# evenrose/CMDIAD

Hardware: AMD Instinct MI355X
Metric: images/sec end-to-end (extract+distill+kNN score) (higher is better)
Workload: dtype bf16; 1 GPU; configs[1]: DINO ViT-B/8 + Point-MAE predict (DoubleRGBPointFeatures: both modalities are extracted, this method has no distillation step at test time; the `mtfi_step` leg times the method that has one), 224x224 RGB + 24576-point clouds (1024 groups x 128), batch 32/GPU, bagel-sized banks (xyz 76518x768, rgb 19129x768); batch_per_gpu=32, rotating_input_batches=4, bank=single, hip_graphs=True, search_operands=bf16 (fp32 accumulate, exact fp32 re-score of the winner), weights=seeded random init (no checkpoints offline)

## Files before the change

cmdiad_amd/csrc/fps.hip:

```cpp
#include "common.h"
#include "launch.h"

namespace {

constexpr int kThreads = 1024;
constexpr int kWaves = kThreads / 64;
constexpr int kMaxRegPoints = 512 * 56;

__device__ __forceinline__ unsigned long long wave_max_u64(unsigned long long v)
{
#pragma unroll
    for (int m = 32; m >= 1; m >>= 1) {
        unsigned long long o = shfl_xor_u64(v, m);
        v = o > v ? o : v;
    }
    return v;
}

__device__ __forceinline__ unsigned long long fps_key(float v, int idx)
{
    return v < 0.0f ? 0ull : (((unsigned long long)__float_as_uint(v) << 32) | (0xFFFFFFFFu - (unsigned)idx));
}

#ifdef CMDIAD_AB_VARIANTS
#include "ab/fps_reg.inc"
#endif


__device__ __forceinline__ unsigned dpp_max_u32(unsigned v)
{
    unsigned o;
    o = (unsigned)__builtin_amdgcn_update_dpp(0, (int)v, 0xB1, 0xF, 0xF, false); v = o > v ? o : v;
    o = (unsigned)__builtin_amdgcn_update_dpp(0, (int)v, 0x4E, 0xF, 0xF, false); v = o > v ? o : v;
    o = (unsigned)__builtin_amdgcn_update_dpp(0, (int)v, 0x141, 0xF, 0xF, false); v = o > v ? o : v;
    o = (unsigned)__builtin_amdgcn_update_dpp(0, (int)v, 0x140, 0xF, 0xF, false); v = o > v ? o : v;
    const unsigned a = __builtin_amdgcn_readlane(v, 0), b = __builtin_amdgcn_readlane(v, 16);
    const unsigned c = __builtin_amdgcn_readlane(v, 32), d = __builtin_amdgcn_readlane(v, 48);
    const unsigned ab = a > b ? a : b, cd = c > d ? c : d;
    return ab > cd ? ab : cd;
}

__device__ __forceinline__ unsigned dpp_min_u32(unsigned v)
{
    unsigned o;
    o = (unsigned)__builtin_amdgcn_update_dpp(0, (int)v, 0xB1, 0xF, 0xF, false); v = o < v ? o : v;
    o = (unsigned)__builtin_amdgcn_update_dpp(0, (int)v, 0x4E, 0xF, 0xF, false); v = o < v ? o : v;
    o = (unsigned)__builtin_amdgcn_update_dpp(0, (int)v, 0x141, 0xF, 0xF, false); v = o < v ? o : v;
    o = (unsigned)__builtin_amdgcn_update_dpp(0, (int)v, 0x140, 0xF, 0xF, false); v = o < v ? o : v;
    const unsigned a = __builtin_amdgcn_readlane(v, 0), b = __builtin_amdgcn_readlane(v, 16);
    const unsigned c = __builtin_amdgcn_readlane(v, 32), d = __builtin_amdgcn_readlane(v, 48);
    const unsigned ab = a < b ? a : b, cd = c < d ? c : d;
    return ab < cd ? ab : cd;
}

template <int kThreads, int PPT, bool TAIL>
__device__ __forceinline__ void fps_pk_body(const float* __restrict__ p, const int n, const int G, int32_t* __restrict__ out,
                                            float* __restrict__ cen, float4* __restrict__ lds_pts, const int lds_cap,
                                            float* __restrict__ temp)
{
    static_assert(PPT % 2 == 0, "two points per packed operation");
    constexpr int kWaves = kThreads / 64, H = PPT / 2, R = PPT * kThreads;
    __shared__ unsigned long long s_key[2][kWaves];
    const int tid = threadIdx.x;

    f32x2 px[H], py[H], pz[H], t[H];
#pragma unroll
    for (int h = 0; h < H; ++h)
#pragma unroll
        for (int e = 0; e < 2; ++e) {
            const int k = (2 * h + e) * kThreads + tid;
            const int kk = max(min(k, n - 1), 0);
            const float x = p[kk * 3 + 0], y = p[kk * 3 + 1], z = p[kk * 3 + 2];
            px[h][e] = x; py[h][e] = y; pz[h][e] = z;
            const float mag = (x * x + y * y) + z * z;
            t[h][e] = (k < n && !(mag <= 1e-3f)) ? 1e10f : -__builtin_inff();
        }
    const int n_lds = TAIL ? min(max(n - R, 0), lds_cap) : 0;
    const int g0 = R + n_lds;
    if constexpr (TAIL) {
        for (int e = tid; e < n_lds; e += kThreads) {
            const int k = R + e;
            const float x = p[k * 3 + 0], y = p[k * 3 + 1], z = p[k * 3 + 2];
            const float mag = (x * x + y * y) + z * z;
            lds_pts[e] = float4{x, y, z, !(mag <= 1e-3f) ? 1e10f : -__builtin_inff()};
        }
        for (int k = g0 + tid; k < n; k += kThreads) {
            const float x = p[k * 3 + 0], y = p[k * 3 + 1], z = p[k * 3 + 2];
            const float mag = (x * x + y * y) + z * z;
            temp[k] = !(mag <= 1e-3f) ? 1e10f : -__builtin_inff();
        }
    }

    int old = 0;
    if (tid == 0 && G > 0) {
        out[0] = 0;
        if (cen) { cen[0] = p[0]; cen[1] = p[1]; cen[2] = p[2]; }
    }
    for (int j = 1; j < G; ++j) {
        const int so = __builtin_amdgcn_readfirstlane(old);
        const float x1 = p[so * 3 + 0], y1 = p[so * 3 + 1], z1 = p[so * 3 + 2];
        const f32x2 X1 = {x1, x1}, Y1 = {y1, y1}, Z1 = {z1, z1};
        int best = 0;
#pragma unroll
        for (int h = 0; h < H; ++h) {
            const f32x2 dx = px[h] - X1, dy = py[h] - Y1, dz = pz[h] - Z1;
            const f32x2 d = (dx * dx + dy * dy) + dz * dz;
            const int a = min((int)__float_as_uint(d[0]), (int)__float_as_uint(t[h][0]));
            const int c = min((int)__float_as_uint(d[1]), (int)__float_as_uint(t[h][1]));
            t[h][0] = __uint_as_float((unsigned)a);
            t[h][1] = __uint_as_float((unsigned)c);
            best = max(best, max(a, c));
        }
        int tb = -1, ti = 0;
        if constexpr (TAIL) {
            for (int e = tid; e < n_lds; e += kThreads) {
                const float4 q = lds_pts[e];
                const float dx = q.x - x1, dy = q.y - y1, dz = q.z - z1;
                const float d = (dx * dx + dy * dy) + dz * dz;
                const int a = min((int)__float_as_uint(d), (int)__float_as_uint(q.w));
                lds_pts[e].w = __uint_as_float((unsigned)a);
                if (a > tb) { tb = a; ti = R + e; }
            }
            for (int k = g0 + tid; k < n; k += kThreads) {
                const float dx = p[k * 3] - x1, dy = p[k * 3 + 1] - y1, dz = p[k * 3 + 2] - z1;
                const float d = (dx * dx + dy * dy) + dz * dz;
                const int a = min((int)__float_as_uint(d), (int)__float_as_uint(temp[k]));
                temp[k] = __uint_as_float((unsigned)a);
                if (a > tb) { tb = a; ti = k; }
            }
        }
        const unsigned wbits = dpp_max_u32((unsigned)max(best, tb));
        int slot = -1;
        unsigned long long lanes = 0ull;
#pragma unroll
        for (int c0 = 0; c0 < PPT; c0 += 8) {
            unsigned long long m[8];
            unsigned long long any = 0ull;
#pragma unroll
            for (int e = 0; e < 8; ++e) {
                const int sl = c0 + e;
                m[e] = sl < PPT ? __ballot(__float_as_uint(t[sl >> 1][sl & 1]) == wbits) : 0ull;
                any |= m[e];
            }
            if (any != 0ull) {
#pragma unroll
                for (int e = 7; e >= 0; --e)
                    if (m[e] != 0ull) { slot = c0 + e; lanes = m[e]; }
                break;
            }
        }
        unsigned long long key = 0ull;
        if (slot >= 0) {
            const int besti = slot * kThreads + (tid & ~63) + (__ffsll((long long)lanes) - 1);
            key = ((unsigned long long)wbits << 32) | (0xFFFFFFFFu - (unsigned)besti);
        } else if constexpr (TAIL) {
            const unsigned cand = dpp_min_u32(tb == (int)wbits ? (unsigned)ti : 0xFFFFFFFFu);
            if (cand != 0xFFFFFFFFu) key = ((unsigned long long)wbits << 32) | (0xFFFFFFFFu - cand);
        }
        const int buf = j & 1;
        if ((tid & 63) == 0) s_key[buf][tid >> 6] = key;
        __syncthreads();
        unsigned long long m = s_key[buf][0];
#pragma unroll
        for (int w = 1; w < kWaves; ++w) {
            const unsigned long long o = s_key[buf][w];
            m = o > m ? o : m;
        }
        old = m == 0ull ? 0 : (int)(0xFFFFFFFFu - (unsigned)(m & 0xFFFFFFFFull));
        if (tid == 0) {
            out[j] = old;
            if (cen) { cen[j * 3 + 0] = p[old * 3 + 0]; cen[j * 3 + 1] = p[old * 3 + 1]; cen[j * 3 + 2] = p[old * 3 + 2]; }
        }
    }
}

template <int kThreads, int PPT>
__global__ __launch_bounds__(kThreads) void fps_pk_kernel(const float* __restrict__ xyz,
                                                          const int32_t* __restrict__ n_valid, int N, int G,
                                                          int32_t* __restrict__ idx_out,
                                                          float* __restrict__ center_out)
{
    const int b = blockIdx.x;
    fps_pk_body<kThreads, PPT, false>(xyz + (size_t)b * N * 3, n_valid ? n_valid[b] : N, G, idx_out + (size_t)b * G,
                                      center_out ? center_out + (size_t)b * G * 3 : nullptr, nullptr, 0, nullptr);
}

constexpr int kRaggedThreads = 512;
constexpr int kMaxLdsPoints = 9728;
__global__ __launch_bounds__(kRaggedThreads) void fps_ragged_kernel(const float* __restrict__ xyz,
                                                                    const int32_t* __restrict__ n_valid, int N, int G,
                                                                    int lds_cap, float* __restrict__ temp_ws,
                                                                    int32_t* __restrict__ idx_out, float* __restrict__ center_out)
{
    extern __shared__ __attribute__((aligned(16))) float4 fps_lds[];
    const int b = blockIdx.x;
    const int n = __builtin_amdgcn_readfirstlane(n_valid ? n_valid[b] : N);
    const float* p = xyz + (size_t)b * N * 3;
    int32_t* out = idx_out + (size_t)b * G;
    float* cen = center_out ? center_out + (size_t)b * G * 3 : nullptr;
    if (n <= kRaggedThreads * 40) fps_pk_body<kRaggedThreads, 40, false>(p, n, G, out, cen, nullptr, 0, nullptr);
    else if (n <= kRaggedThreads * 48) fps_pk_body<kRaggedThreads, 48, false>(p, n, G, out, cen, nullptr, 0, nullptr);
    else if (n <= kRaggedThreads * 56) fps_pk_body<kRaggedThreads, 56, false>(p, n, G, out, cen, nullptr, 0, nullptr);
    else fps_pk_body<kRaggedThreads, 56, true>(p, n, G, out, cen, fps_lds, lds_cap, temp_ws ? temp_ws + (size_t)b * N : nullptr);
}

#ifdef CMDIAD_AB_VARIANTS
__global__ __launch_bounds__(kThreads) void fps_mem_kernel(const float* __restrict__ xyz,
                                                           const int32_t* __restrict__ n_valid, int N, int G,
                                                           float* __restrict__ temp_ws,
                                                           int32_t* __restrict__ idx_out,
                                                           float* __restrict__ center_out)
{
    __shared__ unsigned long long s_key[2][kWaves];
    const int b = blockIdx.x;
    const int tid = threadIdx.x;
    const int n = n_valid ? n_valid[b] : N;
    const float* p = xyz + (size_t)b * N * 3;
    float* temp = temp_ws + (size_t)b * N;
    int32_t* out = idx_out + (size_t)b * G;
    float* cen = center_out ? center_out + (size_t)b * G * 3 : nullptr;

    for (int k = tid; k < n; k += kThreads) {
        const float x = p[k * 3], y = p[k * 3 + 1], z = p[k * 3 + 2];
        const float mag = (x * x + y * y) + z * z;
        temp[k] = !(mag <= 1e-3f) ? 1e10f : -__builtin_inff();
    }
    int old = 0;
    if (tid == 0 && G > 0) {
        out[0] = 0;
        if (cen) { cen[0] = p[0]; cen[1] = p[1]; cen[2] = p[2]; }
    }
    for (int j = 1; j < G; ++j) {
        const int so = __builtin_amdgcn_readfirstlane(old);
        const float x1 = p[so * 3 + 0], y1 = p[so * 3 + 1], z1 = p[so * 3 + 2];
        float best = -1.0f;
        int besti = 0;
        for (int k = tid; k < n; k += kThreads) {
            const float dx = p[k * 3] - x1, dy = p[k * 3 + 1] - y1, dz = p[k * 3 + 2] - z1;
            const float d = (dx * dx + dy * dy) + dz * dz;
            const float d2 = fminf(d, temp[k]);
            temp[k] = d2;
            const bool gt = d2 > best;
            best = gt ? d2 : best;
            besti = gt ? k : besti;
        }
        unsigned long long key = wave_max_u64(fps_key(best, besti));
        const int buf = j & 1;
        if ((tid & 63) == 0) s_key[buf][tid >> 6] = key;
        __syncthreads();
        unsigned long long m = s_key[buf][0];
#pragma unroll
        for (int w = 1; w < kWaves; ++w) {
            const unsigned long long o = s_key[buf][w];
            m = o > m ? o : m;
        }
        old = m == 0ull ? 0 : (int)(0xFFFFFFFFu - (unsigned)(m & 0xFFFFFFFFull));
        if (tid == 0) {
            out[j] = old;
            if (cen) { cen[j * 3 + 0] = p[old * 3 + 0]; cen[j * 3 + 1] = p[old * 3 + 1]; cen[j * 3 + 2] = p[old * 3 + 2]; }
        }
    }
}

#endif

}

struct FpsWs { float* min_d; size_t total; };
static FpsWs fps_layout(void* base, int B, int N)
{
    Carve c(base);
    return {c.take<float>(N > kMaxRegPoints + kMaxLdsPoints ? (size_t)B * (size_t)N : 0), c.total()};
}

extern "C" size_t cmdiad_fps_workspace_bytes(int B, int N) { return fps_layout(nullptr, B, N).total; }

extern "C" int cmdiad_fps(const float* xyz, const int32_t* n_valid, int B, int N, int G, int32_t* idx_out,
                          float* center_out, void* workspace, size_t workspace_bytes, cmdiad_stream_t stream)
{
    CMDIAD_REQUIRE(xyz && idx_out, CMDIAD_ERR_ARG, "cmdiad_fps: null pointer");
    CMDIAD_REQUIRE(B >= 0 && N > 0 && G >= 0, CMDIAD_ERR_ARG, "cmdiad_fps: bad sizes B=%d N=%d G=%d", B, N, G);
    if (B == 0 || G == 0) return CMDIAD_OK;
    hipStream_t s = (hipStream_t)stream;
#ifdef CMDIAD_AB_VARIANTS
    const bool pk = !env_is("CMDIAD_FPS_PK", '0');
    const bool ragged_ok = !env_is("CMDIAD_FPS_RAGGED", '0');
#define FPS_LAUNCH(T, P)                                                                                                      \
    do {                                                                                                                      \
        if (pk) hipLaunchKernelGGL((fps_pk_kernel<T, P>), dim3(B), dim3(T), 0, s, xyz, n_valid, N, G, idx_out, center_out);   \
        else hipLaunchKernelGGL((fps_reg_kernel<T, P>), dim3(B), dim3(T), 0, s, xyz, n_valid, N, G, idx_out, center_out);     \
    } while (0)
#else
    const bool ragged_ok = true;
#define FPS_LAUNCH(T, P) hipLaunchKernelGGL((fps_pk_kernel<T, P>), dim3(B), dim3(T), 0, s, xyz, n_valid, N, G, idx_out, center_out)
#endif
    const bool ragged = ragged_ok && N > 1024 * 16 && (n_valid != nullptr || N > kMaxRegPoints);
    if (ragged) {
        const int lds_cap = N > kMaxRegPoints ? (N - kMaxRegPoints < kMaxLdsPoints ? N - kMaxRegPoints : kMaxLdsPoints) : 0;
        const FpsWs L = fps_layout(workspace, B, N);
        if (const int rc = workspace_ok("cmdiad_fps", workspace, workspace_bytes, L.total)) return rc;
        if (const int rc = launch_lds<fps_ragged_kernel>("cmdiad_fps", dim3(B), dim3(kRaggedThreads), (size_t)lds_cap * sizeof(float4), s, xyz, n_valid,
                                                         N, G, lds_cap, L.total ? L.min_d : nullptr, idx_out, center_out))
            return rc;
    }
    else if (N <= 1024 * 4) FPS_LAUNCH(1024, 4);
    else if (N <= 1024 * 8) FPS_LAUNCH(1024, 8);
    else if (N <= 1024 * 16) FPS_LAUNCH(1024, 16);
    else if (N <= 512 * 40) FPS_LAUNCH(512, 40);
    else if (N <= 512 * 48) FPS_LAUNCH(512, 48);
    else if (N <= 512 * 56) FPS_LAUNCH(512, 56);
#undef FPS_LAUNCH
    else {
#ifdef CMDIAD_AB_VARIANTS
        Carve c(workspace);
        float* const min_d = c.take<float>((size_t)B * (size_t)N);
        if (const int rc = workspace_ok("cmdiad_fps", workspace, workspace_bytes, c.total())) return rc;
        hipLaunchKernelGGL(fps_mem_kernel, dim3(B), dim3(kThreads), 0, s, xyz, n_valid, N, G, min_d, idx_out, center_out);
#else
        cmdiad_set_error("cmdiad_fps: unreachable dispatch (N=%d)", N);
        return CMDIAD_ERR_ARG;
#endif
    }
    CMDIAD_CHECK_LAUNCH();
    return CMDIAD_OK;
}
```

Baseline: 1550 images/s.

## Add spatially bucketed FPS with bounding-box lower-bound pruning for large clouds

Adds a pruned farthest-point-sampling body. Points are sorted into Morton-ordered 2D grid cells via an LDS histogram, scan and scatter, so each register slot holds a spatially coherent bucket. Each bucket keeps a bounding box and its running max distance, which lets whole buckets skip the distance update when the box lower bound cannot lower their max. This targets the per-iteration O(N) distance work for 24576-point clouds, which goes through the ragged path since N > 16K. In exchange it adds setup passes, extra LDS and divergent per-slot summary work.

```diff
diff --git a/cmdiad_amd/csrc/fps.hip b/cmdiad_amd/csrc/fps.hip
--- a/cmdiad_amd/csrc/fps.hip
+++ b/cmdiad_amd/csrc/fps.hip
@@ -1,3 +1,4 @@
+#include "block_scan.h"
 #include "common.h"
 #include "launch.h"
 
@@ -185,8 +186,253 @@
                                       center_out ? center_out + (size_t)b * G * 3 : nullptr, nullptr, 0, nullptr);
 }
 
+constexpr int kPruneThreads = 512, kPruneWaves = kPruneThreads / 64;
+constexpr int kPruneCells = 64 * 64;
+constexpr int kPruneHist = kPruneThreads * 9;
+constexpr size_t kPruneLdsBytes = (size_t)kMaxRegPoints * sizeof(uint16_t) + (size_t)kPruneHist * sizeof(int);
+
+__device__ __forceinline__ unsigned f2ord(float f)
+{
+    const unsigned b = __float_as_uint(f);
+    return b ^ ((b >> 31) ? 0xFFFFFFFFu : 0x80000000u);
+}
+__device__ __forceinline__ float ord2f(unsigned u) { return __uint_as_float(u ^ ((u >> 31) ? 0x80000000u : 0xFFFFFFFFu)); }
+
+__device__ __forceinline__ unsigned dpp8_max_u32(unsigned v)
+{
+    unsigned o;
+    o = (unsigned)__builtin_amdgcn_update_dpp(0, (int)v, 0xB1, 0xF, 0xF, false); v = o > v ? o : v;
+    o = (unsigned)__builtin_amdgcn_update_dpp(0, (int)v, 0x4E, 0xF, 0xF, false); v = o > v ? o : v;
+    o = (unsigned)__builtin_amdgcn_update_dpp(0, (int)v, 0x141, 0xF, 0xF, false); v = o > v ? o : v;
+    return (unsigned)__builtin_amdgcn_readfirstlane((int)v);
+}
+__device__ __forceinline__ unsigned dpp8_min_u32(unsigned v)
+{
+    unsigned o;
+    o = (unsigned)__builtin_amdgcn_update_dpp(0, (int)v, 0xB1, 0xF, 0xF, false); v = o < v ? o : v;
+    o = (unsigned)__builtin_amdgcn_update_dpp(0, (int)v, 0x4E, 0xF, 0xF, false); v = o < v ? o : v;
+    o = (unsigned)__builtin_amdgcn_update_dpp(0, (int)v, 0x141, 0xF, 0xF, false); v = o < v ? o : v;
+    return (unsigned)__builtin_amdgcn_readfirstlane((int)v);
+}
+
+template <class F>
+__device__ __forceinline__ void fps_each_point(const float* __restrict__ p, const int n, F f)
+{
+    constexpr int U = 8;
+    const int tid = threadIdx.x;
+    for (int k0 = 0; k0 < n; k0 += U * kPruneThreads) {
+        float x[U], y[U], z[U];
+#pragma unroll
+        for (int e = 0; e < U; ++e) {
+            const int kk = max(min(k0 + e * kPruneThreads + tid, n - 1), 0);
+            x[e] = p[kk * 3 + 0]; y[e] = p[kk * 3 + 1]; z[e] = p[kk * 3 + 2];
+        }
+#pragma unroll
+        for (int e = 0; e < U; ++e) {
+            const int k = k0 + e * kPruneThreads + tid;
+            if (k < n) f(k, x[e], y[e], z[e]);
+        }
+    }
+}
+
+__device__ __forceinline__ void fps_bucket_summary(const int s, const float ts, const float xs, const float ys,
+                                                   const float zs, const uint16_t* __restrict__ wave_order, float& sbmax, unsigned& sbidx,
+                                                   float& scx, float& scy, float& scz)
+{
+    const int lane = threadIdx.x & 63;
+    const unsigned tb = __float_as_uint(ts);
+    const unsigned m = dpp_max_u32((unsigned)max((int)tb, 0));
+    const unsigned long long lanes = __ballot(tb == m);
+    float nb = -__builtin_inff(), cx = 0.0f, cy = 0.0f, cz = 0.0f;
+    unsigned ni = 0u;
+    if (lanes != 0ull) {
+        int L;
+        if (lanes & (lanes - 1ull)) {
+            const unsigned oi = tb == m ? (unsigned)wave_order[s * (kPruneWaves * 64) + lane] : 0xFFFFFFFFu;
+            ni = dpp_min_u32(oi);
+            L = __ffsll((long long)__ballot(oi == ni)) - 1;
+        } else {
+            L = __ffsll((long long)lanes) - 1;
+            ni = (unsigned)__builtin_amdgcn_readfirstlane((int)wave_order[s * (kPruneWaves * 64) + L]);
+        }
+        nb = __uint_as_float(m);
+        cx = __uint_as_float((unsigned)__builtin_amdgcn_readlane((int)__float_as_uint(xs), L));
+        cy = __uint_as_float((unsigned)__builtin_amdgcn_readlane((int)__float_as_uint(ys), L));
+        cz = __uint_as_float((unsigned)__builtin_amdgcn_readlane((int)__float_as_uint(zs), L));
+    }
+    if (lane == s) { sbmax = nb; sbidx = ni; scx = cx; scy = cy; scz = cz; }
+}
+
+template <int PPT>
+__device__ __forceinline__ void fps_prune_body(const float* __restrict__ p, const int n, const int G, int32_t* __restrict__ out,
+                                               float* __restrict__ cen, void* __restrict__ lds)
+{
+    static_assert(PPT % 8 == 0 && PPT <= 64, "slots are walked eight at a time; one summary lane per slot");
+    static_assert(PPT * kPruneThreads <= kMaxRegPoints && kMaxRegPoints <= 65536, "16-bit rank table");
+    constexpr int T = kPruneThreads, W = kPruneWaves;
+    __shared__ float s_box[W][6];
+    __shared__ int s_scan[W];
+    __shared__ float4 s_win[2][W];
+    __shared__ float s_wz[2][W];
+    uint16_t* const order = (uint16_t*)lds;
+    int* const hist = (int*)((char*)lds + (size_t)kMaxRegPoints * sizeof(uint16_t));
+    const int tid = threadIdx.x, lane = tid & 63, wave = __builtin_amdgcn_readfirstlane(tid >> 6);
+    const float inf = __builtin_inff();
+    const uint16_t* const wave_order = order + wave * 64;
+
+    float lo0 = inf, lo1 = inf, lo2 = inf, hi0 = -inf, hi1 = -inf, hi2 = -inf;
+    fps_each_point(p, n, [&](int, float x, float y, float z) {
+        const float mag = (x * x + y * y) + z * z;
+        if (!(mag <= 1e-3f)) {
+            lo0 = fminf(lo0, x); lo1 = fminf(lo1, y); lo2 = fminf(lo2, z);
+            hi0 = fmaxf(hi0, x); hi1 = fmaxf(hi1, y); hi2 = fmaxf(hi2, z);
+        }
+    });
+#pragma unroll
+    for (int m = 32; m >= 1; m >>= 1) {
+        lo0 = fminf(lo0, __shfl_xor(lo0, m, 64)); lo1 = fminf(lo1, __shfl_xor(lo1, m, 64)); lo2 = fminf(lo2, __shfl_xor(lo2, m, 64));
+        hi0 = fmaxf(hi0, __shfl_xor(hi0, m, 64)); hi1 = fmaxf(hi1, __shfl_xor(hi1, m, 64)); hi2 = fmaxf(hi2, __shfl_xor(hi2, m, 64));
+    }
+    if (lane == 0) {
+        s_box[wave][0] = lo0; s_box[wave][1] = lo1; s_box[wave][2] = lo2;
+        s_box[wave][3] = hi0; s_box[wave][4] = hi1; s_box[wave][5] = hi2;
+    }
+    for (int i = tid; i < kPruneHist; i += T) hist[i] = 0;
+    __syncthreads();
+#pragma unroll
+    for (int w = 0; w < W; ++w) {
+        lo0 = fminf(lo0, s_box[w][0]); lo1 = fminf(lo1, s_box[w][1]); lo2 = fminf(lo2, s_box[w][2]);
+        hi0 = fmaxf(hi0, s_box[w][3]); hi1 = fmaxf(hi1, s_box[w][4]); hi2 = fmaxf(hi2, s_box[w][5]);
+    }
+    const float e0 = hi0 - lo0, e1 = hi1 - lo1, e2 = hi2 - lo2;
+    const int drop = (e2 <= e0 && e2 <= e1) ? 2 : (e1 <= e0 ? 1 : 0);
+    const float ulo = drop == 0 ? lo1 : lo0, uext = drop == 0 ? e1 : e0;
+    const float vlo = drop == 2 ? lo1 : lo2, vext = drop == 2 ? e1 : e2;
+    const float uinv = uext > 0.0f ? 64.0f / uext : 0.0f, vinv = vext > 0.0f ? 64.0f / vext : 0.0f;
+    auto cell = [&](float x, float y, float z) -> int {
+        const float mag = (x * x + y * y) + z * z;
+        if (mag <= 1e-3f) return kPruneCells;
+        const float u = drop == 0 ? y : x, v = drop == 2 ? y : z;
+        unsigned iu = (unsigned)(int)fminf(fmaxf((u - ulo) * uinv, 0.0f), 63.0f);
+        unsigned iv = (unsigned)(int)fminf(fmaxf((v - vlo) * vinv, 0.0f), 63.0f);
+        iu = (iu | (iu << 4)) & 0x0F0Fu; iu = (iu | (iu << 2)) & 0x3333u; iu = (iu | (iu << 1)) & 0x5555u;
+        iv = (iv | (iv << 4)) & 0x0F0Fu; iv = (iv | (iv << 2)) & 0x3333u; iv = (iv | (iv << 1)) & 0x5555u;
+        return (int)(iu | (iv << 1));
+    };
+
+    fps_each_point(p, n, [&](int, float x, float y, float z) { atomicAdd(&hist[cell(x, y, z)], 1); });
+    __syncthreads();
+    {
+        int cnt[9], sum = 0, total;
+#pragma unroll
+        for (int e = 0; e < 9; ++e) { cnt[e] = hist[tid * 9 + e]; sum += cnt[e]; }
+        int run = block_excl_scan<W>(sum, s_scan, total);
+#pragma unroll
+        for (int e = 0; e < 9; ++e) { hist[tid * 9 + e] = run; run += cnt[e]; }
+    }
+    __syncthreads();
+    fps_each_point(p, n, [&](int k, float x, float y, float z) { order[atomicAdd(&hist[cell(x, y, z)], 1)] = (uint16_t)k; });
+    __syncthreads();
+
+    float px[PPT], py[PPT], pz[PPT], t[PPT];
+#pragma unroll
+    for (int s = 0; s < PPT; ++s) {
+        const int r = s * (W * 64) + wave * 64 + lane;
+        const int k = n > 0 ? (int)order[min(r, n - 1)] : 0;
+        const float x = p[k * 3 + 0], y = p[k * 3 + 1], z = p[k * 3 + 2];
+        px[s] = x; py[s] = y; pz[s] = z;
+        const float mag = (x * x + y * y) + z * z;
+        t[s] = (r < n && !(mag <= 1e-3f)) ? 1e10f : -inf;
+    }
+    float slo0 = inf, slo1 = inf, slo2 = inf, shi0 = -inf, shi1 = -inf, shi2 = -inf, sbmax = -inf, scx = 0.0f, scy = 0.0f, scz = 0.0f;
+    unsigned sbidx = 0u;
+#pragma unroll
+    for (int s = 0; s < PPT; ++s) {
+        const bool v = t[s] > 0.0f;
+        const float a0 = ord2f(dpp_min_u32(f2ord(v ? px[s] : inf))), b0 = ord2f(dpp_max_u32(f2ord(v ? px[s] : -inf)));
+        const float a1 = ord2f(dpp_min_u32(f2ord(v ? py[s] : inf))), b1 = ord2f(dpp_max_u32(f2ord(v ? py[s] : -inf)));
+        const float a2 = ord2f(dpp_min_u32(f2ord(v ? pz[s] : inf))), b2 = ord2f(dpp_max_u32(f2ord(v ? pz[s] : -inf)));
+        if (lane == s) { slo0 = a0; slo1 = a1; slo2 = a2; shi0 = b0; shi1 = b1; shi2 = b2; }
+        fps_bucket_summary(s, t[s], px[s], py[s], pz[s], wave_order, sbmax, sbidx, scx, scy, scz);
+        __builtin_amdgcn_sched_barrier(0);
+    }
+
+    const float p0x = p[0], p0y = p[1], p0z = p[2];
+    float sx = p0x, sy = p0y, sz = p0z;
+    if (tid == 0 && G > 0) {
+        out[0] = 0;
+        if (cen) { cen[0] = p0x; cen[1] = p0y; cen[2] = p0z; }
+    }
+    for (int j = 1; j < G; ++j) {
+        const float dx = fminf(fmaxf(sx, slo0), shi0) - sx, dy = fminf(fmaxf(sy, slo1), shi1) - sy, dz = fminf(fmaxf(sz, slo2), shi2) - sz;
+        const float lb = (dx * dx + dy * dy) + dz * dz;
+        const unsigned long long act = __ballot(lb < sbmax);
+#pragma unroll
+        for (int c0 = 0; c0 < PPT; c0 += 8) {
+            if (((act >> c0) & 0xFFull) == 0ull) continue;
+#pragma unroll
+            for (int e = 0; e < 8; ++e) {
+                const int s = c0 + e;
+                if (!((act >> s) & 1ull)) continue;
+                const float ex = px[s] - sx, ey = py[s] - sy, ez = pz[s] - sz;
+                const float d = (ex * ex + ey * ey) + ez * ez;
+                t[s] = __uint_as_float((unsigned)min((int)__float_as_uint(d), (int)__float_as_uint(t[s])));
+                fps_bucket_summary(s, t[s], px[s], py[s], pz[s], wave_order, sbmax, sbidx, scx, scy, scz);
+            }
+        }
+        const unsigned sb = __float_as_uint(sbmax);
+        const unsigned wm = dpp_max_u32((unsigned)max((int)sb, 0));
+        const bool mt = sb == wm;
+        const unsigned long long ml = __ballot(mt);
+        unsigned kv = 0u, wi = 0u;
+        float wx = 0.0f, wy = 0.0f, wz = 0.0f;
+        if (ml != 0ull) {
+            int L;
+            if (ml & (ml - 1ull)) {
+                const unsigned oi = mt ? sbidx : 0xFFFFFFFFu;
+                wi = dpp_min_u32(oi);
+                L = __ffsll((long long)__ballot(oi == wi)) - 1;
+            } else {
+                L = __ffsll((long long)ml) - 1;
+                wi = (unsigned)__builtin_amdgcn_readlane((int)sbidx, L);
+            }
+            kv = wm + 1u;
+            wx = __uint_as_float((unsigned)__builtin_amdgcn_readlane((int)__float_as_uint(scx), L));
+            wy = __uint_as_float((unsigned)__builtin_amdgcn_readlane((int)__float_as_uint(scy), L));
+            wz = __uint_as_float((unsigned)__builtin_amdgcn_readlane((int)__float_as_uint(scz), L));
+        }
+        const int buf = j & 1;
+        if (lane == 0) { s_win[buf][wave] = float4{__uint_as_float(kv), __uint_as_float(wi), wx, wy}; s_wz[buf][wave] = wz; }
+        __syncthreads();
+        const float4 en = s_win[buf][lane & (W - 1)];
+        const float enz = s_wz[buf][lane & (W - 1)];
+        const unsigned ev = __float_as_uint(en.x), ei = __float_as_uint(en.y);
+        const unsigned best = dpp8_max_u32(ev);
+        int old = 0;
+        sx = p0x; sy = p0y; sz = p0z;
+        if (best != 0u) {
+            unsigned long long mm = __ballot(ev == best) & 0xFFull;
+            if (mm & (mm - 1ull)) {
+                const unsigned oi = ev == best ? ei : 0xFFFFFFFFu;
+                mm = __ballot(oi == dpp8_min_u32(oi)) & 0xFFull;
+            }
+            const int L = __ffsll((long long)mm) - 1;
+            old = __builtin_amdgcn_readlane((int)ei, L);
+            sx = __uint_as_float((unsigned)__builtin_amdgcn_readlane((int)__float_as_uint(en.z), L));
+            sy = __uint_as_float((unsigned)__builtin_amdgcn_readlane((int)__float_as_uint(en.w), L));
+            sz = __uint_as_float((unsigned)__builtin_amdgcn_readlane((int)__float_as_uint(enz), L));
+        }
+        if (tid == 0) {
+            out[j] = old;
+            if (cen) { cen[j * 3 + 0] = sx; cen[j * 3 + 1] = sy; cen[j * 3 + 2] = sz; }
+        }
+    }
+}
+
 constexpr int kRaggedThreads = 512;
 constexpr int kMaxLdsPoints = 9728;
+static_assert(kRaggedThreads == kPruneThreads, "one block shape for every body of fps_ragged_kernel");
+template <bool PRUNE>
 __global__ __launch_bounds__(kRaggedThreads) void fps_ragged_kernel(const float* __restrict__ xyz,
                                                                     const int32_t* __restrict__ n_valid, int N, int G,
                                                                     int lds_cap, float* __restrict__ temp_ws,
@@ -198,10 +444,17 @@
     const float* p = xyz + (size_t)b * N * 3;
     int32_t* out = idx_out + (size_t)b * G;
     float* cen = center_out ? center_out + (size_t)b * G * 3 : nullptr;
-    if (n <= kRaggedThreads * 40) fps_pk_body<kRaggedThreads, 40, false>(p, n, G, out, cen, nullptr, 0, nullptr);
-    else if (n <= kRaggedThreads * 48) fps_pk_body<kRaggedThreads, 48, false>(p, n, G, out, cen, nullptr, 0, nullptr);
-    else if (n <= kRaggedThreads * 56) fps_pk_body<kRaggedThreads, 56, false>(p, n, G, out, cen, nullptr, 0, nullptr);
-    else fps_pk_body<kRaggedThreads, 56, true>(p, n, G, out, cen, fps_lds, lds_cap, temp_ws ? temp_ws + (size_t)b * N : nullptr);
+    if constexpr (PRUNE) {
+        if (n <= kRaggedThreads * 40) fps_prune_body<40>(p, n, G, out, cen, fps_lds);
+        else if (n <= kRaggedThreads * 48) fps_prune_body<48>(p, n, G, out, cen, fps_lds);
+        else if (n <= kRaggedThreads * 56) fps_prune_body<56>(p, n, G, out, cen, fps_lds);
+        else fps_pk_body<kRaggedThreads, 56, true>(p, n, G, out, cen, fps_lds, lds_cap, temp_ws ? temp_ws + (size_t)b * N : nullptr);
+    } else {
+        if (n <= kRaggedThreads * 40) fps_pk_body<kRaggedThreads, 40, false>(p, n, G, out, cen, nullptr, 0, nullptr);
+        else if (n <= kRaggedThreads * 48) fps_pk_body<kRaggedThreads, 48, false>(p, n, G, out, cen, nullptr, 0, nullptr);
+        else if (n <= kRaggedThreads * 56) fps_pk_body<kRaggedThreads, 56, false>(p, n, G, out, cen, nullptr, 0, nullptr);
+        else fps_pk_body<kRaggedThreads, 56, true>(p, n, G, out, cen, fps_lds, lds_cap, temp_ws ? temp_ws + (size_t)b * N : nullptr);
+    }
 }
 
 #ifdef CMDIAD_AB_VARIANTS
@@ -285,23 +538,28 @@
 #ifdef CMDIAD_AB_VARIANTS
     const bool pk = !env_is("CMDIAD_FPS_PK", '0');
     const bool ragged_ok = !env_is("CMDIAD_FPS_RAGGED", '0');
+    const bool prune_ok = pk;
 #define FPS_LAUNCH(T, P)                                                                                                      \
     do {                                                                                                                      \
         if (pk) hipLaunchKernelGGL((fps_pk_kernel<T, P>), dim3(B), dim3(T), 0, s, xyz, n_valid, N, G, idx_out, center_out);   \
         else hipLaunchKernelGGL((fps_reg_kernel<T, P>), dim3(B), dim3(T), 0, s, xyz, n_valid, N, G, idx_out, center_out);     \
     } while (0)
 #else
-    const bool ragged_ok = true;
+    const bool ragged_ok = true, prune_ok = true;
 #define FPS_LAUNCH(T, P) hipLaunchKernelGGL((fps_pk_kernel<T, P>), dim3(B), dim3(T), 0, s, xyz, n_valid, N, G, idx_out, center_out)
 #endif
+    const bool prune = ragged_ok && prune_ok && !env_is("CMDIAD_FPS_PRUNE", '0') && (N > 1024 * 16 || env_is("CMDIAD_FPS_PRUNE", '1'));
     const bool ragged = ragged_ok && N > 1024 * 16 && (n_valid != nullptr || N > kMaxRegPoints);
-    if (ragged) {
+    if (prune || ragged) {
         const int lds_cap = N > kMaxRegPoints ? (N - kMaxRegPoints < kMaxLdsPoints ? N - kMaxRegPoints : kMaxLdsPoints) : 0;
+        const size_t tier_bytes = (size_t)lds_cap * sizeof(float4);
         const FpsWs L = fps_layout(workspace, B, N);
         if (const int rc = workspace_ok("cmdiad_fps", workspace, workspace_bytes, L.total)) return rc;
-        if (const int rc = launch_lds<fps_ragged_kernel>("cmdiad_fps", dim3(B), dim3(kRaggedThreads), (size_t)lds_cap * sizeof(float4), s, xyz, n_valid,
-                                                         N, G, lds_cap, L.total ? L.min_d : nullptr, idx_out, center_out))
-            return rc;
+        const int rc = prune ? launch_lds<fps_ragged_kernel<true>>("cmdiad_fps", dim3(B), dim3(kRaggedThreads), tier_bytes > kPruneLdsBytes ? tier_bytes : kPruneLdsBytes,
+                                                                   s, xyz, n_valid, N, G, lds_cap, L.total ? L.min_d : nullptr, idx_out, center_out)
+                             : launch_lds<fps_ragged_kernel<false>>("cmdiad_fps", dim3(B), dim3(kRaggedThreads), tier_bytes, s, xyz, n_valid, N, G, lds_cap,
+                                                                    L.total ? L.min_d : nullptr, idx_out, center_out);
+        if (rc) return rc;
     }
     else if (N <= 1024 * 4) FPS_LAUNCH(1024, 4);
     else if (N <= 1024 * 8) FPS_LAUNCH(1024, 8);
```

Result: no change. 1539 images/s (-0.7%).
